# chao9527/Paddle_infer

Measured on AMD Instinct MI355X. Metric: tokens/sec (node) GPT-3 1.3B Fleet hybrid-parallel at 1/2/4/8 MI355X, higher is better.
Workload: dtype bf16; 1 GPU; model=GPT-3 1.3B, global_batch=96, seq_len=1024, parallelism=dp1, micro_batch_per_dp_rank=96, params=1313722368, optimizer=AdamW fp32 master, api=fleet.init/distributed_model/distributed_optimizer

## Files before the change

### paddle_infer_amd/csrc/kernels/layernorm.hip

```cpp
#include "common.h"

#include <cstdlib>
#include <type_traits>

namespace {

enum { DT_F32 = 0, DT_BF16 = 1, DT_F16 = 2 };

template <int DT>
struct IO16 {
  typedef unsigned short T;
  typedef u16x8 Raw;
  static __device__ __forceinline__ float cv(unsigned short v) {
    if (DT == DT_BF16) return bf2f(v);
    return (float)__builtin_bit_cast(_Float16, v);
  }
  static __device__ __forceinline__ unsigned short cvt(float f) {
    if (DT == DT_BF16) return f2bf(f);
    return __builtin_bit_cast(unsigned short, (_Float16)f);
  }
  static __device__ __forceinline__ Raw ldraw(const T* p) { return *reinterpret_cast<const Raw*>(p); }
  static __device__ __forceinline__ float el(const Raw& r, int j) { return cv(r[j]); }
  static __device__ __forceinline__ void load8(const T* p, float* v) {
    u16x8 r = *reinterpret_cast<const u16x8*>(p);
// ... 501 lines not shown
    __syncthreads();
    if (rp == 0) {
#pragma unroll
      for (int i = 0; i < NV; ++i) {
        const int vi = vcol(i);
        if (vi >= nvec) continue;
        f32x4 a, b;
#pragma unroll
        for (int j = 0; j < 4; ++j) {
          a[j] = (q == 0 ? dg[i][j] : (q == 1 ? db[i][j] : dbi[i][j])) + cmb[half][lane][i * 8 + j];
          b[j] = (q == 0 ? dg[i][4 + j] : (q == 1 ? db[i][4 + j] : dbi[i][4 + j])) + cmb[half][lane][i * 8 + 4 + j];
        }
        *reinterpret_cast<f32x4*>(outs[q] + srow + vi * 8) = a;
        *reinterpret_cast<f32x4*>(outs[q] + srow + vi * 8 + 4) = b;
      }
    }
    __syncthreads();
  }
}


#define LN_BWD_PAIR_PARAMS                                                                         \
  const typename IO<DT>::T *__restrict__ dy, const typename IO<DT>::T *__restrict__ h,             \
      const typename IO<DT>::T *__restrict__ gamma, const float *__restrict__ mean_in,             \
      const float *__restrict__ rstd_in, const typename IO<DT>::T *__restrict__ dres_in,           \
      typename IO<DT>::T *__restrict__ dres, typename IO<DT>::T *__restrict__ dx,                  \
      float *__restrict__ acc_dg, float *__restrict__ acc_db, float *__restrict__ acc_dbias, int rows, \
      int N, float p_drop, uint64_t seed, uint64_t offset, int rms
#define LN_BWD_PAIR_ARGS dy, h, gamma, mean_in, rstd_in, dres_in, dres, dx, acc_dg, acc_db, acc_dbias, \
                         rows, N, p_drop, seed, offset, rms
template <int DT>
__global__ __launch_bounds__(256) __attribute__((amdgpu_waves_per_eu(3, 3))) void ln_bwd_pair_kernel(
    LN_BWD_PAIR_PARAMS) {
  ln_bwd_pair_body<DT>(LN_BWD_PAIR_ARGS);
}
template <int DT>
__global__ __launch_bounds__(256) void ln_bwd_pair_kernel_f32(LN_BWD_PAIR_PARAMS) {
  ln_bwd_pair_body<DT>(LN_BWD_PAIR_ARGS);
}
#undef LN_BWD_PAIR_PARAMS
#undef LN_BWD_PAIR_ARGS
template <int NV, int DT>
__global__ __launch_bounds__(512) void ln_bwd_wide_kernel(
    const typename IO<DT>::T* __restrict__ dy, const typename IO<DT>::T* __restrict__ h,
    const typename IO<DT>::T* __restrict__ gamma, const float* __restrict__ mean_in,
    const float* __restrict__ rstd_in, const typename IO<DT>::T* __restrict__ dres_in,
    typename IO<DT>::T* __restrict__ dres, typename IO<DT>::T* __restrict__ dx,
    float* __restrict__ acc_dg, float* __restrict__ acc_db, float* __restrict__ acc_dbias,
    int rows, int N, float p_drop, uint64_t seed, uint64_t offset, int rms) {
  __shared__ float red[16];
  const int nvec = N >> 3;
  float dg[NV][8], db[NV][8], dbi[NV][8];
#pragma unroll
  for (int i = 0; i < NV; ++i)
#pragma unroll
    for (int j = 0; j < 8; ++j) { dg[i][j] = 0.f; db[i][j] = 0.f; dbi[i][j] = 0.f; }
  const float keep_scale = p_drop > 0.f ? 1.f / (1.f - p_drop) : 1.f;
  for (int row = blockIdx.x; row < rows; row += gridDim.x)
    ln_bwd_row<NV, DT, 512, 8>(dy, h, gamma, mean_in[row], rstd_in[row], dres_in, dres, dx,
                               (size_t)row * N, threadIdx.x, nvec, N, p_drop, keep_scale, seed,
                               offset, rms, dg, db, dbi, red);
  float* outs[3] = {acc_dg, acc_db, acc_dbias};
  const size_t srow = (size_t)blockIdx.x * N;
#pragma unroll
  for (int q = 0; q < 3; ++q) {
    if (!outs[q]) continue;
#pragma unroll
    for (int i = 0; i < NV; ++i) {
      const int vi = i * 512 + threadIdx.x;
      if (vi < nvec) {
        f32x4 a, b;
#pragma unroll
        for (int j = 0; j < 4; ++j) {
          a[j] = q == 0 ? dg[i][j] : (q == 1 ? db[i][j] : dbi[i][j]);
          b[j] = q == 0 ? dg[i][4 + j] : (q == 1 ? db[i][4 + j] : dbi[i][4 + j]);
        }
        *reinterpret_cast<f32x4*>(outs[q] + srow + vi * 8) = a;
        *reinterpret_cast<f32x4*>(outs[q] + srow + vi * 8 + 4) = b;
      }
    }
  }
}

__global__ __launch_bounds__(256) void slab_reduce_kernel(float* __restrict__ s0, float* __restrict__ s1,
                                                          float* __restrict__ s2, float* __restrict__ a0,
                                                          float* __restrict__ a1, float* __restrict__ a2,
                                                          int G, int N) {
  const int q = blockIdx.z;
  const float* slab = q == 0 ? s0 : (q == 1 ? s1 : s2);
  float* acc = q == 0 ? a0 : (q == 1 ? a1 : a2);
  if (!slab) return;
  const int c4 = blockIdx.x * 1024 + threadIdx.x * 4;
  if (c4 >= N) return;
  const int g0 = blockIdx.y * 16, g1 = min(g0 + 16, G);
  f32x4 s = {0.f, 0.f, 0.f, 0.f};
#pragma unroll 4
  for (int g = g0; g < g1; ++g) s += *reinterpret_cast<const f32x4*>(slab + (size_t)g * N + c4);
#pragma unroll
  for (int j = 0; j < 4; ++j) atomicAdd(acc + c4 + j, s[j]);
}

template <int DT>
__global__ __launch_bounds__(256) void col_sum_kernel(const float* __restrict__ part, int G, int N,
                                                     typename IO<DT>::T* __restrict__ out,
                                                     int accumulate) {
  const int cl = threadIdx.x & 63, rg = threadIdx.x >> 6;
  const int col = blockIdx.x * 64 + cl;
  float s = 0.f;
  if (col < N)
    for (int g = rg; g < G; g += 4) s += part[(size_t)g * N + col];
  __shared__ float red[4][64];
  red[rg][cl] = s;
  __syncthreads();
  if (rg == 0 && col < N) {
    float t = red[0][cl] + red[1][cl] + red[2][cl] + red[3][cl];
    if (accumulate) t += IO<DT>::load1(out + col);
    IO<DT>::store1(out + col, t);
  }
}

template <int DT>
int launch_fwd(const void* x, const void* bias, const void* residual, const void* gamma,
               const void* beta, void* y, void* residual_out, float* mean, float* rstd, int rows,
               int N, float eps, float p, uint64_t seed, uint64_t off, int rms, hipStream_t st) {
  typedef typename IO<DT>::T T;
#define ROW_ARGS (const T*)x, (const T*)bias, (const T*)residual, (const T*)gamma, (const T*)beta, \
                 (T*)y, (T*)residual_out, mean, rstd, N, eps, p, seed, off, rms
  if (N > 4096) {
    switch ((N / 8 + 511) / 512) {
      case 2: hipLaunchKernelGGL((ln_fwd_row_kernel<8, 2, DT>), dim3(rows), dim3(512), 0, st, ROW_ARGS); break;
      case 3: hipLaunchKernelGGL((ln_fwd_row_kernel<8, 3, DT>), dim3(rows), dim3(512), 0, st, ROW_ARGS); break;
      case 4: hipLaunchKernelGGL((ln_fwd_row_kernel<8, 4, DT>), dim3(rows), dim3(512), 0, st, ROW_ARGS); break;
      default: return (int)hipErrorInvalidValue;
    }
    return (int)hipGetLastError();
  }
  static const int row_max = [] {
    const char* e = getenv("PIAMD_LN_ROW_MAX");
    return e ? atoi(e) : 512;
  }();
  if (rows <= row_max) {
    switch ((N / 8 + 255) / 256) {
      case 1: hipLaunchKernelGGL((ln_fwd_row_kernel<4, 1, DT>), dim3(rows), dim3(256), 0, st, ROW_ARGS); break;
      case 2: hipLaunchKernelGGL((ln_fwd_row_kernel<4, 2, DT>), dim3(rows), dim3(256), 0, st, ROW_ARGS); break;
      default: return (int)hipErrorInvalidValue;
    }
    return (int)hipGetLastError();
  }
#undef ROW_ARGS
  const int nv = (N / 8 + 63) / 64;
  dim3 grid((rows + 3) / 4), block(256);
#define LNF(NVV)                                                                                  \
  hipLaunchKernelGGL((ln_fwd_kernel<NVV, DT>), grid, block, 0, st, (const T*)x, (const T*)bias, \
                     (const T*)residual, (const T*)gamma, (const T*)beta, (T*)y,               \
                     (T*)residual_out, mean, rstd, rows, N, eps, p, seed, off, rms);           \
  break;
  switch (nv) {
    case 1: LNF(1)
    case 2: LNF(2)
    case 3: LNF(3)
    case 4: LNF(4)
    case 5: case 6: LNF(6)
    case 7: case 8: LNF(8)
    default: return (int)hipErrorInvalidValue;
  }
#undef LNF
  return (int)hipGetLastError();
}

static inline bool bwd_pair(int N) {
  static const bool on = [] {
    const char* e = getenv("PIAMD_LN_BWD_PAIR");
    return !(e && e[0] == '0');
  }();
  return on && N > 1024 && N <= 2048;
}

static inline int bwd_grid(int rows, int N) {
  if (bwd_pair(N)) {
    const int g = (rows + 1) / 2;
    return g > 768 ? 768 : (g < 1 ? 1 : g);
  }
// ... 27 lines not shown
    else
      hipLaunchKernelGGL((ln_bwd_pair_kernel<DT>), grid, block, 0, st, BWD_ARGS);
    return (int)hipGetLastError();
  }
  switch ((N / 8 + 63) / 64) {
    case 1: hipLaunchKernelGGL((ln_bwd_kernel<1, DT>), grid, block, 0, st, BWD_ARGS); break;
    case 2: hipLaunchKernelGGL((ln_bwd_kernel<2, DT>), grid, block, 0, st, BWD_ARGS); break;
    case 3: hipLaunchKernelGGL((ln_bwd_kernel<3, DT>), grid, block, 0, st, BWD_ARGS); break;
    case 4: hipLaunchKernelGGL((ln_bwd_kernel<4, DT>), grid, block, 0, st, BWD_ARGS); break;
    default: return (int)hipErrorInvalidValue;
  }
#undef BWD_ARGS
  return (int)hipGetLastError();
}

template <int DT>
__global__ __launch_bounds__(256) void col_sum4_kernel(const float* __restrict__ part, int G, int N,
                                                      typename IO<DT>::T* __restrict__ out,
                                                      int accumulate) {
  const int q = threadIdx.x & 7, rg = threadIdx.x >> 3;
  const int col = blockIdx.x * 32 + 4 * q;
  f32x4 s = {0.f, 0.f, 0.f, 0.f};
  if (col < N) {
#pragma unroll 4
    for (int g = rg; g < G; g += 32) s += *reinterpret_cast<const f32x4*>(part + (size_t)g * N + col);
  }
  __shared__ f32x4 red[32][9];
  red[rg][q] = s;
  __syncthreads();
  if (threadIdx.x < 32) {
    const int qq = threadIdx.x >> 2, j = threadIdx.x & 3, c = blockIdx.x * 32 + threadIdx.x;
    if (c < N) {
      float t = 0.f;
#pragma unroll 8
      for (int r = 0; r < 32; ++r) t += red[r][qq][j];
      if (accumulate) t += IO<DT>::load1(out + c);
      IO<DT>::store1(out + c, t);
    }
  }
}

template <int DT>
void launch_colsum_out(const float* part, int G, int N, void* out, int acc, hipStream_t st) {
  if (G >= 64 && N % 4 == 0 && ((uintptr_t)part & 15) == 0) {
    hipLaunchKernelGGL((col_sum4_kernel<DT>), dim3((N + 31) / 32), dim3(256), 0, st, part, G, N,
                       (typename IO<DT>::T*)out, acc);
    return;
  }
  hipLaunchKernelGGL((col_sum_kernel<DT>), dim3((N + 63) / 64), dim3(256), 0, st, part, G, N,
                     (typename IO<DT>::T*)out, acc);
}

}

PIAMD_EXPORT int piamd_layernorm_fwd(int dtype, const void* x, const void* bias,
                                     const void* residual, const void* gamma, const void* beta,
                                     void* y, void* residual_out, float* mean, float* rstd,
                                     int rows, int N, float eps, float p_drop, uint64_t seed,
                                     uint64_t offset, int flags, hipStream_t stream) {
  if (N % 8 != 0 || N > 16384 || dtype < 0 || dtype > 2) return (int)hipErrorInvalidValue;
  if (rows == 0) return 0;
  const int rms = flags & 1;
#define FWD(D) launch_fwd<D>(x, bias, residual, gamma, beta, y, residual_out, mean, rstd, rows, N, \
                             eps, p_drop, seed, offset, rms, stream)
  return dtype == DT_BF16 ? FWD(DT_BF16) : (dtype == DT_F16 ? FWD(DT_F16) : FWD(DT_F32));
#undef FWD
}

PIAMD_EXPORT long long piamd_layernorm_bwd_ws(int rows, int N) {
  return 3LL * ((long long)bwd_grid(rows, N) * N + N);
}

PIAMD_EXPORT int piamd_layernorm_bwd(int dtype, const void* dy, const void* h, const void* gamma,
                                     const float* mean, const float* rstd, const void* dres_in,
                                     void* dres, void* dx, void* dgamma, void* dbeta, void* dbias,
                                     float* ws, int rows, int N, float p_drop, uint64_t seed,
                                     uint64_t offset, int accum_mask, int flags,
                                     hipStream_t stream) {
  if (N % 8 != 0 || N > 16384 || dtype < 0 || dtype > 2) return (int)hipErrorInvalidValue;
  if (rows == 0) return 0;
  const int rms = flags & 1;
  const int G = bwd_grid(rows, N);
  void* outs[3] = {dgamma, dbeta, dbias};
  float *slab[3], *acc[3];
  for (int q = 0; q < 3; ++q) {
    slab[q] = outs[q] ? ws + (size_t)q * G * N : nullptr;
    acc[q] = outs[q] ? ws + (size_t)3 * G * N + (size_t)q * N : nullptr;
    if (outs[q]) (void)hipMemsetAsync(acc[q], 0, sizeof(float) * N, stream);
  }
#define BWD(D) launch_bwd<D>(dy, h, gamma, mean, rstd, dres_in, dres, dx, slab[0], slab[1], slab[2], \
                             rows, N, p_drop, seed, offset, rms, stream)
  int e = dtype == DT_BF16 ? BWD(DT_BF16) : (dtype == DT_F16 ? BWD(DT_F16) : BWD(DT_F32));
#undef BWD
  if (e) return e;
  if (dgamma || dbeta || dbias)
    hipLaunchKernelGGL(slab_reduce_kernel, dim3((N + 1023) / 1024, (G + 15) / 16, 3), dim3(256), 0,
                       stream, slab[0], slab[1], slab[2], acc[0], acc[1], acc[2], G, N);
  for (int q = 0; q < 3; ++q) {
    if (!outs[q]) continue;
    const int a = (accum_mask >> q) & 1;
    if (dtype == DT_BF16) launch_colsum_out<DT_BF16>(acc[q], 1, N, outs[q], a, stream);
    else if (dtype == DT_F16) launch_colsum_out<DT_F16>(acc[q], 1, N, outs[q], a, stream);
    else launch_colsum_out<DT_F32>(acc[q], 1, N, outs[q], a, stream);
  }
  return (int)hipGetLastError();
}

template <int DT>
__global__ __launch_bounds__(256) void rowsum_partial_kernel(const typename IO<DT>::T* __restrict__ x,
                                                            int rows, int N,
                                                            float* __restrict__ part) {
  const int col = blockIdx.y * 256 + threadIdx.x;
  if (col >= N) return;
  float s = 0.f;
  for (int r = blockIdx.x; r < rows; r += gridDim.x) {
    s += IO<DT>::load1(x + (size_t)r * N + col);
  }
  part[(size_t)blockIdx.x * N + col] = s;
}

__global__ __launch_bounds__(256) void rowsum_partial_bf16x8_kernel(const bf16_t* __restrict__ x,
                                                                    int rows, int N,
                                                                    float* __restrict__ part) {
  const int c8 = blockIdx.y * 256 + threadIdx.x;
  if (c8 * 8 >= N) return;
  float s[8] = {0, 0, 0, 0, 0, 0, 0, 0};
  constexpr int U = 4;
  for (int r0 = blockIdx.x; r0 < rows; r0 += U * gridDim.x) {
    u16x8 v[U];
#pragma unroll
    for (int u = 0; u < U; ++u) {
      const int r = min(r0 + u * (int)gridDim.x, rows - 1);
      v[u] = reinterpret_cast<const u16x8*>(x + (size_t)r * N)[c8];
    }
#pragma unroll
    for (int u = 0; u < U; ++u)
      if (r0 + u * (int)gridDim.x < rows)
#pragma unroll
        for (int j = 0; j < 8; ++j) s[j] += bf2f(v[u][j]);
  }
  float* p = part + (size_t)blockIdx.x * N + c8 * 8;
#pragma unroll
  for (int j = 0; j < 8; ++j) p[j] = s[j];
}

PIAMD_EXPORT int piamd_colsum(int dtype, const void* x, void* out, float* part, int G, int rows,
                              int N, int accumulate, hipStream_t stream) {
  if (rows == 0) return 0;
  if (dtype < 0 || dtype > 2) return (int)hipErrorInvalidValue;
  dim3 grid(G, (N + 255) / 256), block(256);
  if (dtype == DT_BF16 && N % 8 == 0)
    hipLaunchKernelGGL(rowsum_partial_bf16x8_kernel, dim3(G, (N / 8 + 255) / 256), block, 0, stream,
                       (const bf16_t*)x, rows, N, part);
  else if (dtype == DT_BF16)
    hipLaunchKernelGGL((rowsum_partial_kernel<DT_BF16>), grid, block, 0, stream, (const bf16_t*)x,
                       rows, N, part);
  else if (dtype == DT_F16)
    hipLaunchKernelGGL((rowsum_partial_kernel<DT_F16>), grid, block, 0, stream,
                       (const unsigned short*)x, rows, N, part);
  else
    hipLaunchKernelGGL((rowsum_partial_kernel<DT_F32>), grid, block, 0, stream, (const float*)x,
                       rows, N, part);
  if (dtype == DT_BF16) launch_colsum_out<DT_BF16>(part, G, N, out, accumulate, stream);
  else if (dtype == DT_F16) launch_colsum_out<DT_F16>(part, G, N, out, accumulate, stream);
  else launch_colsum_out<DT_F32>(part, G, N, out, accumulate, stream);
  return (int)hipGetLastError();
}

PIAMD_EXPORT int piamd_colsum_parts(int dtype, const float* part, int G, int N, void* out, int accumulate,
                                    hipStream_t stream) {
  if (G <= 0 || N <= 0) return 0;
  if (dtype == DT_BF16) launch_colsum_out<DT_BF16>(part, G, N, out, accumulate, stream);
  else if (dtype == DT_F16) launch_colsum_out<DT_F16>(part, G, N, out, accumulate, stream);
  else if (dtype == DT_F32) launch_colsum_out<DT_F32>(part, G, N, out, accumulate, stream);
  else return (int)hipErrorInvalidValue;
  return (int)hipGetLastError();
}
```

### paddle_infer_amd/csrc/kernels/xent.hip

```cpp
#include "common.h"

namespace {

__device__ __forceinline__ void online_update(float& m, float& s, float x) {
  if (x > m) { s = s * __expf(m - x) + 1.f; m = x; }
  else s += __expf(x - m);
}
__device__ __forceinline__ void online_merge(float& m, float& s, float m2, float s2) {
  float M = fmaxf(m, m2);
  if (M == -INFINITY) { m = M; s = 0.f; return; }
  s = s * __expf(m - M) + s2 * __expf(m2 - M);
  m = M;
}

template <int DT>
__global__ __launch_bounds__(256) void xent_stats_kernel(
    const void* __restrict__ logits, const long long* __restrict__ labels, int V,
    long long vocab_start, int ignore_index, float* __restrict__ out_max,
    float* __restrict__ out_sum, float* __restrict__ out_target) {
  constexpr bool BF16 = DT != 0, F16 = DT == 2;
  const int row = blockIdx.x;
  const size_t base = (size_t)row * V;
  float m = -INFINITY, s = 0.f;
  if (BF16 && (V % 8) == 0) {
    const u16x8* p = reinterpret_cast<const u16x8*>((const bf16_t*)logits + base);
    for (int i = threadIdx.x; i < V / 8; i += 256) {
      u16x8 r = p[i];
      float x[8], lm = -INFINITY;
#pragma unroll
      for (int j = 0; j < 8; ++j) { x[j] = h2f<F16>(r[j]); lm = fmaxf(lm, x[j]); }
      float ls = 0.f;
#pragma unroll
      for (int j = 0; j < 8; ++j) ls += __expf(x[j] - lm);
      online_merge(m, s, lm, ls);
    }
  } else {
    for (int i = threadIdx.x; i < V; i += 256) {
      float x = BF16 ? h2f<F16>(((const bf16_t*)logits)[base + i]) : ((const float*)logits)[base + i];
      online_update(m, s, x);
    }
  }
#pragma unroll
  for (int o = 32; o > 0; o >>= 1) {
    float m2 = __shfl_xor(m, o, 64), s2 = __shfl_xor(s, o, 64);
    online_merge(m, s, m2, s2);
  }
  __shared__ float sm[4], ss[4];
  const int lane = threadIdx.x & 63, w = threadIdx.x >> 6;
  if (lane == 0) { sm[w] = m; ss[w] = s; }
  __syncthreads();
  if (threadIdx.x == 0) {
    float M = sm[0], S = ss[0];
    for (int i = 1; i < 4; ++i) online_merge(M, S, sm[i], ss[i]);
    out_max[row] = M;
    out_sum[row] = S;
    const long long lab = labels[row];
    float t = 0.f;
    if (lab != ignore_index && lab >= vocab_start && lab < vocab_start + V) {
      const size_t k = base + (size_t)(lab - vocab_start);
      t = BF16 ? h2f<F16>(((const bf16_t*)logits)[k]) : ((const float*)logits)[k];
    }
    out_target[row] = t;
  }
}

template <int DT>
__global__ __launch_bounds__(256) void xent_bwd_kernel(
    const void* __restrict__ logits, const long long* __restrict__ labels,
    const float* __restrict__ lse, const float* __restrict__ dloss, float dloss_scalar, int V,
    long long vocab_start, int ignore_index, void* __restrict__ grad) {
  constexpr bool BF16 = DT != 0, F16 = DT == 2;
  const int row = blockIdx.x;
  const size_t base = (size_t)row * V;
  const long long lab = labels[row];
  const float L = lse[row];
  const float d = lab == ignore_index ? 0.f : (dloss ? dloss[row] : dloss_scalar);
  const long long tl = lab - vocab_start;
  if (BF16 && (V % 8) == 0) {
    const u16x8* p = reinterpret_cast<const u16x8*>((const bf16_t*)logits + base);
    u16x8* q = reinterpret_cast<u16x8*>((bf16_t*)grad + base);
    for (int i = threadIdx.x; i < V / 8; i += 256) {
      u16x8 r = p[i], o;
#pragma unroll
      for (int j = 0; j < 8; ++j) {
        float g = __expf(h2f<F16>(r[j]) - L);
        if ((long long)(i * 8 + j) == tl) g -= 1.f;
        o[j] = f2h<F16>(g * d);
      }
      q[i] = o;
    }
  } else {
    for (int i = threadIdx.x; i < V; i += 256) {
      float x = BF16 ? h2f<F16>(((const bf16_t*)logits)[base + i]) : ((const float*)logits)[base + i];
      float g = __expf(x - L);
      if ((long long)i == tl) g -= 1.f;
      g *= d;
      if (BF16) ((bf16_t*)grad)[base + i] = f2h<F16>(g);
      else ((float*)grad)[base + i] = g;
    }
  }
}

}

PIAMD_EXPORT int piamd_xent_stats(int dtype, const void* logits, const long long* labels, int rows,
                                  int V, long long vocab_start, int ignore_index, float* out_max,
                                  float* out_sum, float* out_target, hipStream_t stream) {
  if (rows == 0) return 0;
#define XS(D)                                                                                     \
  hipLaunchKernelGGL((xent_stats_kernel<D>), dim3(rows), dim3(256), 0, stream, logits, labels, V, \
                     vocab_start, ignore_index, out_max, out_sum, out_target)
  if (dtype == 1) XS(1); else if (dtype == 2) XS(2); else if (dtype == 0) XS(0);
  else return (int)hipErrorInvalidValue;
#undef XS
  return (int)hipGetLastError();
}

PIAMD_EXPORT int piamd_xent_bwd(int dtype, const void* logits, const long long* labels,
                                const float* lse, const float* dloss, float dloss_scalar, int rows,
                                int V, long long vocab_start, int ignore_index, void* grad,
                                hipStream_t stream) {
  if (rows == 0) return 0;
#define XB(D)                                                                                     \
  hipLaunchKernelGGL((xent_bwd_kernel<D>), dim3(rows), dim3(256), 0, stream, logits, labels, lse, \
                     dloss, dloss_scalar, V, vocab_start, ignore_index, grad)
  if (dtype == 1) XB(1); else if (dtype == 2) XB(2); else if (dtype == 0) XB(0);
  else return (int)hipErrorInvalidValue;
#undef XB
  return (int)hipGetLastError();
}
```

### paddle_infer_amd/models/gpt.py

```python
from __future__ import annotations

import math
from dataclasses import dataclass, field

import torch
import torch.nn.functional as F

from ..nn.layer.base import Layer, LayerList
from ..nn import initializer as I
from ..ops import fused_add_layer_norm, flash_attention_packed, bias_act, softmax_cross_entropy
from ..ops.linear import (_use_transposed, fused_mlp, fused_mlp_supported, mm_nt, transposed,
                          wgrad_into)
from ..ops.linear import linear as _linear
from ..ops.embedding import embedding as ops_embedding
from ..distributed.fleet.mp_layers import (ColumnParallelLinear, RowParallelLinear,
                                           VocabParallelEmbedding, c_identity)


@dataclass
class GPTConfig:
    vocab_size: int = 50304
    hidden_size: int = 2048
    num_layers: int = 24
    num_heads: int = 16
    num_kv_heads: int | None = None
    ffn_hidden_size: int | None = None
    max_position_embeddings: int = 1024
    hidden_dropout_prob: float = 0.1
    attention_probs_dropout_prob: float = 0.0
    layer_norm_eps: float = 1e-5
    initializer_range: float = 0.02
    activation: str = "gelu_tanh"
    tie_word_embeddings: bool = True
    dtype: str = "bfloat16"
    recompute: bool = False
    extra: dict = field(default_factory=dict)

    @property
    def head_dim(self):
        return self.hidden_size // self.num_heads

    @property
    def ffn(self):
        return self.ffn_hidden_size or 4 * self.hidden_size


PRESETS = {
    "gpt3-tiny": dict(vocab_size=1024, hidden_size=256, num_layers=2, num_heads=4,
                      max_position_embeddings=256),
    "gpt3-125m": dict(hidden_size=768, num_layers=12, num_heads=12),
    "gpt3-350m": dict(hidden_size=1024, num_layers=24, num_heads=16),
    "gpt3-760m": dict(hidden_size=1536, num_layers=24, num_heads=16),
    "gpt3-1.3b": dict(hidden_size=2048, num_layers=24, num_heads=16),
    "gpt3-2.7b": dict(hidden_size=2560, num_layers=32, num_heads=32),
    "gpt3-6.7b": dict(hidden_size=4096, num_layers=32, num_heads=32, max_position_embeddings=2048),
    "gpt3-13b": dict(hidden_size=5120, num_layers=40, num_heads=40, max_position_embeddings=2048),
}


def gpt_config(name: str, **over) -> GPTConfig:
    kw = dict(PRESETS[name])
    kw.update(over)
    return GPTConfig(**kw)


def _mp_size(group):
    import torch.distributed as dist
    return dist.get_world_size(group) if group is not None else 1


class GPTAttention(Layer):
    def __init__(self, cfg: GPTConfig, mp_group=None, layer_idx=0):
        super().__init__(dtype=cfg.dtype)
        t = _mp_size(mp_group)
        self.cfg = cfg
        self.heads = cfg.num_heads // t
        self.kv_heads = (cfg.num_kv_heads or cfg.num_heads) // t
        self.head_dim = cfg.head_dim
        qkv_out = (cfg.num_heads + 2 * (cfg.num_kv_heads or cfg.num_heads)) * cfg.head_dim
        std = cfg.initializer_range
        self.qkv_proj = ColumnParallelLinear(cfg.hidden_size, qkv_out, gather_output=False,
                                             mp_group=mp_group, dtype=cfg.dtype,
                                             weight_attr=I.Normal(0.0, std))
        self.out_proj = RowParallelLinear(cfg.hidden_size, cfg.hidden_size, input_is_parallel=True,
                                          mp_group=mp_group, dtype=cfg.dtype,
                                          weight_attr=I.Normal(0.0, std / math.sqrt(2 * cfg.num_layers)))
        self.mp_group = mp_group

    def forward(self, y):
        B, S, _ = y.shape
        x = c_identity(y, self.mp_group)
        qkv = _linear(x, self.qkv_proj.weight, self.qkv_proj.bias)
        qkv = qkv.view(B, S, self.heads + 2 * self.kv_heads, self.head_dim)
# ... 82 lines not shown
        return w + pe


class _LMHeadFn(torch.autograd.Function):

    @staticmethod
    def forward(ctx, y, w):
        shp = y.shape
        y2 = y.reshape(-1, shp[-1])
        ctx.save_for_backward(y2, w)
        ctx.shp = shp
        return mm_nt(y2.contiguous(), w).view(*shp[:-1], w.shape[0])

    @staticmethod
    def backward(ctx, dl):
        y2, w = ctx.saved_tensors
        dl2 = dl.reshape(-1, w.shape[0])
        dl2 = dl2.contiguous()
        if _use_transposed(dl2, w) or (dl2.is_cuda and dl2.dtype == w.dtype
                                       and dl2.dtype in (torch.bfloat16, torch.float16)):
            dy = mm_nt(dl2, transposed(w)).view(ctx.shp)
        else:
            dy = torch.mm(dl2, w).view(ctx.shp)
        mg = getattr(w, "main_grad", None)
        if mg is not None:
            wgrad_into(mg, dl2, y2)
            return dy, None
        return dy, wgrad_into(torch.zeros_like(w), dl2, y2)


class GPTModel(Layer):
    def __init__(self, cfg: GPTConfig, mp_group=None):
        super().__init__(dtype=cfg.dtype)
        self.cfg = cfg
        self.mp_group = mp_group
        self.embeddings = GPTEmbeddings(cfg, mp_group)
        self.layers = LayerList([GPTDecoderLayer(cfg, mp_group, i) for i in range(cfg.num_layers)])
        self.final_ln = _LNParams(cfg)

    def forward(self, input_ids, position_ids=None):
        emb = self.embeddings(input_ids, position_ids)
        p = self.cfg.hidden_dropout_prob if self.training else 0.0
        h = None
        out, bias = emb, None
        for layer in self.layers:
            if self.cfg.recompute and self.training:
                from ..distributed.fleet.recompute import recompute
                h, out = recompute(lambda hh, oo, bb, _l=layer: _l(hh, oo, bb)[:2], h, out, bias)
                bias = None if getattr(self, "_zero3", False) else layer.mlp.fc2.bias
            else:
                h, out, bias = layer(h, out, bias)
        y, _ = fused_add_layer_norm(out, h, self.final_ln.weight, self.final_ln.bias,
                                    self.cfg.layer_norm_eps, bias, p, self.training)
        return y


class GPTForPretraining(Layer):
    def __init__(self, cfg: GPTConfig, mp_group=None):
        super().__init__(dtype=cfg.dtype)
        self.cfg = cfg
        self.gpt = GPTModel(cfg, mp_group)
        self.mp_group = mp_group
        if not cfg.tie_word_embeddings:
            self.lm_head = self.create_parameter(
                [cfg.vocab_size // _mp_size(mp_group), cfg.hidden_size],
                default_initializer=I.Normal(0.0, cfg.initializer_range))

    @property
    def _stage3_persistent(self):
        return ["gpt.embeddings.word_embeddings"] if self.cfg.tie_word_embeddings else []

    def head_weight(self):
        if self.cfg.tie_word_embeddings:
            return self.gpt.embeddings.word_embeddings.weight
        return self.lm_head

    def forward(self, input_ids, labels=None, position_ids=None, loss_mask=None):
        y = self.gpt(input_ids, position_ids)
        y = c_identity(y, self.mp_group)
        logits = _LMHeadFn.apply(y, self.head_weight())
        if labels is None:
            return logits
        group = self.mp_group if _mp_size(self.mp_group) > 1 else None
        loss = softmax_cross_entropy(logits, labels, group=group, inplace_backward=True)
        if loss_mask is not None:
            lm = loss_mask.reshape(-1).float()
            return (loss.reshape(-1) * lm).sum() / lm.sum()
        return loss.float().mean()


class GPTPretrainingCriterion(Layer):

    def __init__(self, mp_group=None):
        super().__init__()
        self.mp_group = mp_group

    def forward(self, logits, labels, loss_mask=None):
        group = self.mp_group if _mp_size(self.mp_group) > 1 else None
        loss = softmax_cross_entropy(logits, labels, group=group)
        if loss_mask is None:
            return loss.float().mean()
        lm = loss_mask.reshape(-1).float()
        return (loss.reshape(-1).float() * lm).sum() / lm.sum()


def gpt_flops_per_token(cfg: GPTConfig, seq_len: int) -> float:
    h, L, V = cfg.hidden_size, cfg.num_layers, cfg.vocab_size
    per_layer = 2 * (3 * h * h + h * h + 2 * h * cfg.ffn) + 2 * 2 * seq_len * h / 2
    return 3 * (L * per_layer + 2 * h * V)


def _qkv_cols(cfg: GPTConfig):
    hk = cfg.num_kv_heads or cfg.num_heads
    D = cfg.head_dim
    return cfg.num_heads * D, hk * D


def shard_gpt_state_dict(full: dict, cfg: GPTConfig, rank: int, world: int) -> dict:
    out = {}
    qc, kc = _qkv_cols(cfg)
    for k, v in full.items():
        if k.endswith("qkv_proj.weight") or k.endswith("qkv_proj.bias"):
            q, kk, vv = v.split([qc, kc, kc], dim=-1)
            out[k] = torch.cat([t.chunk(world, dim=-1)[rank] for t in (q, kk, vv)], dim=-1).clone()
        elif k.endswith("fc1.weight") or k.endswith("fc1.bias"):
            out[k] = v.chunk(world, dim=-1)[rank].clone()
        elif k.endswith("out_proj.weight") or k.endswith("fc2.weight"):
            out[k] = v.chunk(world, dim=0)[rank].clone()
        elif k.endswith("word_embeddings.weight") or k == "lm_head":
            out[k] = v.chunk(world, dim=0)[rank].clone()
        else:
            out[k] = v.clone()
    return out


def merge_gpt_state_dicts(shards: list, cfg: GPTConfig) -> dict:
    world = len(shards)
    qc, kc = _qkv_cols(cfg)
    out = {}
    for k in shards[0]:
        vs = [s[k] for s in shards]
        if k.endswith("qkv_proj.weight") or k.endswith("qkv_proj.bias"):
            parts = [v.split([qc // world, kc // world, kc // world], dim=-1) for v in vs]
            out[k] = torch.cat([torch.cat([p[i] for p in parts], dim=-1) for i in range(3)], dim=-1)
        elif k.endswith("fc1.weight") or k.endswith("fc1.bias"):
            out[k] = torch.cat(vs, dim=-1)
        elif k.endswith("out_proj.weight") or k.endswith("fc2.weight") or \
                k.endswith("word_embeddings.weight") or k == "lm_head":
            out[k] = torch.cat(vs, dim=0)
        else:
            out[k] = vs[0]
    return out


class GPTEmbeddingPipe(GPTEmbeddings):

    @property
    def weight(self):
        return self.word_embeddings.weight

    def forward(self, input_ids, position_ids=None):
        return super().forward(input_ids, position_ids)


class GPTDecoderLayerPipe(GPTDecoderLayer):

# ... 89 lines not shown
```

### paddle_infer_amd/ops/__init__.py

```python
from .norm import layer_norm, fused_add_layer_norm, rms_norm, fused_add_rms_norm
from .attention import (flash_attention, flash_attention_packed, attention_reference,
                        flash_attention_varlen)
from .activation import bias_act, gelu, dropout, fused_softmax_mask
from .loss import softmax_cross_entropy
from .optim import adamw_flat, momentum_flat, sumsq
from . import _lib
from .inference import (qkv_prep, decode_attention, weight_quantize, weight_dequantize,
                        weight_only_linear, llm_int8_linear, int8_linear,
                        quantize_rows)


def _make_recordable():
    from ..static.framework import recordable
    g = globals()
    for name, ty in (("layer_norm", "layer_norm"), ("fused_add_layer_norm", "skip_layernorm"),
                     ("rms_norm", "rms_norm"), ("flash_attention", "flash_attn"),
                     ("flash_attention_packed", "flash_attn_packed"), ("bias_act", "fused_bias_act"),
                     ("gelu", "gelu"), ("dropout", "dropout"), ("fused_softmax_mask", "softmax_mask_fuse"),
                     ("softmax_cross_entropy", "softmax_with_cross_entropy"),
                     ("weight_only_linear", "weight_only_linear")):
        g[name] = recordable(ty)(g[name])


_make_recordable()
```

### paddle_infer_amd/ops/_lib.py

```python
from __future__ import annotations

import ctypes
import os
import threading

import torch

from .. import _build

_LIB = None
_LOCK = threading.Lock()

c_void_p, c_int, c_float, c_ll, c_u64 = (ctypes.c_void_p, ctypes.c_int, ctypes.c_float,
                                         ctypes.c_longlong, ctypes.c_uint64)

_SIGS = {
    "piamd_layernorm_fwd": [c_int, c_void_p, c_void_p, c_void_p, c_void_p, c_void_p, c_void_p,
                            c_void_p, c_void_p, c_void_p, c_int, c_int, c_float, c_float, c_u64,
                            c_u64, c_int, c_void_p],
    "piamd_layernorm_bwd": [c_int, c_void_p, c_void_p, c_void_p, c_void_p, c_void_p, c_void_p,
                            c_void_p, c_void_p, c_void_p, c_void_p, c_void_p, c_void_p, c_int, c_int,
                            c_float, c_u64, c_u64, c_int, c_int, c_void_p],
    "piamd_colsum": [c_int, c_void_p, c_void_p, c_void_p, c_int, c_int, c_int, c_int, c_void_p],
    "piamd_adamw_flat": [c_void_p, c_void_p, c_void_p, c_void_p, c_int, c_void_p, c_ll, c_float,
                         c_void_p, c_float, c_float, c_float, c_float, c_float, c_float, c_void_p,
                         c_float, c_void_p],
    "piamd_momentum_flat": [c_void_p, c_void_p, c_void_p, c_int, c_void_p, c_ll, c_float,
                            c_void_p, c_float, c_float, c_int, c_void_p, c_void_p],
    "piamd_sumsq": [c_void_p, c_int, c_ll, c_void_p, c_void_p, c_int, c_void_p],
    "piamd_xent_stats": [c_int, c_void_p, c_void_p, c_int, c_int, c_ll, c_int, c_void_p, c_void_p,
                         c_void_p, c_void_p],
    "piamd_xent_bwd": [c_int, c_void_p, c_void_p, c_void_p, c_void_p, c_float, c_int, c_int, c_ll,
                       c_int, c_void_p, c_void_p],
    "piamd_bias_act_fwd": [c_int, c_int, c_void_p, c_void_p, c_void_p, c_void_p, c_ll, c_int, c_void_p],
    "piamd_bias_act_bwd_grid": [c_int],
    "piamd_bias_act_bwd": [c_int, c_int, c_void_p, c_void_p, c_void_p, c_void_p, c_void_p, c_void_p,
                           c_int, c_int, c_int, c_void_p],
    "piamd_softmax_fwd": [c_int, c_void_p, c_void_p, c_int, c_int, c_void_p, c_int, c_int, c_float,
                          c_void_p],
    "piamd_softmax_bwd": [c_int, c_void_p, c_void_p, c_void_p, c_int, c_int, c_float, c_void_p],
    "piamd_dropout": [c_int, c_void_p, c_void_p, c_ll, c_float, c_u64, c_u64, c_void_p],
    "piamd_qkv_prep": [c_void_p, c_ll, c_void_p, c_void_p, c_void_p, c_void_p, c_int, c_int,
                       c_int, c_int, c_int, c_int, c_int, c_int, c_float, c_void_p],
    "piamd_decode_attn": [c_void_p, c_ll, c_void_p, c_int, c_int, c_int, c_float, c_void_p,
                          c_void_p, c_void_p, c_int, c_int, c_int, c_int, c_int, c_int, c_int,
                          c_void_p, c_ll, c_float, c_void_p, c_void_p, c_void_p, c_ll, c_void_p],
    "piamd_wo_gemm": [c_int, c_void_p, c_ll, c_void_p, c_void_p, c_void_p, c_void_p, c_ll,
                      c_void_p, c_void_p, c_int, c_int, c_int, c_int, c_int, c_void_p],
    "piamd_conv_wprep": [c_int, c_int, c_void_p, c_void_p, c_void_p, c_int, c_int, c_int, c_int, c_int,
                         c_int, c_int, c_void_p],
    "piamd_wo_gemm_ex": [c_int, c_void_p, c_ll, c_void_p, c_void_p, c_void_p, c_void_p, c_ll,
                         c_void_p, c_void_p, c_int, c_int, c_int, c_int, c_int, c_void_p,
                         c_void_p, c_float, c_void_p, c_ll, c_void_p],
    "piamd_wo_dequant": [c_int, c_void_p, c_void_p, c_void_p, c_int, c_int, c_void_p],
}


_RESTYPES = {"piamd_layernorm_bwd_ws": ctypes.c_longlong, "piamd_dconv2d_wgrad_parts": ctypes.c_longlong,
             "piamd_group_norm_ws": ctypes.c_longlong}


class FaArgs(ctypes.Structure):
    _fields_ = ([(n, c_void_p) for n in ("q", "k", "v", "o", "lse", "dout", "delta", "dq", "dk", "dv",
                                        "mask", "cu_q", "cu_k")]
                + [(n, c_int) for n in ("B", "Sq", "Sk", "Hq", "Hk", "D", "ltot", "causal")]
                + [(n, c_ll) for n in ("sqb", "sqs", "sqh", "skb", "sks", "skh", "svb", "svs", "svh",
                                       "sob", "sos", "soh", "smb", "smh", "smq")]
                + [("scale", ctypes.c_float), ("p_drop", ctypes.c_float), ("seed", c_u64),
                   ("offset", c_u64), ("map", c_int), ("ds", c_void_p)])


class MegaArgs(ctypes.Structure):
    _fields_ = ([("layers", c_void_p)] + [(n, c_int) for n in ("nl", "maxS", "nsplit", "act")]
                + [("eps", ctypes.c_float), ("scale_log2", ctypes.c_float)]
                + [(n, c_void_p) for n in ("resid", "rbuf", "qn", "kvn", "part", "h", "bar", "err",
                                        "pos", "trace")] + [("late_dma", c_int), ("loader", c_int)]
                + [("rot", c_int), ("neox", c_int), ("log2_base", ctypes.c_float), ("w8", c_int),
                   ("nb", c_int), ("mm", c_int)])


_SIGS["piamd_decode_mega"] = [ctypes.POINTER(MegaArgs), c_int, c_int, c_int, c_int, c_int, c_void_p]
_SIGS["piamd_decode_mega_shape_supported"] = [c_int] * 7
_SIGS["piamd_decode_mega_batch_supported"] = [c_int] * 8
_SIGS["piamd_decode_mega_variant_supported"] = [c_int] * 9


class HeadArgs(ctypes.Structure):
    _fields_ = ([(n, c_void_p) for n in ("y", "g", "b")] + [("eps", ctypes.c_float), ("V", c_int)]
                + [(n, c_void_p) for n in ("w", "best", "cnt", "out", "done")]
                + [("eos", ctypes.c_longlong), ("pad", ctypes.c_longlong)]
                + [(n, c_void_p) for n in ("pos", "tok", "wemb", "pemb")]
                + [("P", c_int), ("resid", c_void_p)])


_SIGS["piamd_decode_head_greedy"] = [ctypes.POINTER(HeadArgs), c_int, c_void_p]
_SIGS["piamd_decode_mega_supported"] = []
_SIGS["piamd_fa_fwd"] = [ctypes.POINTER(FaArgs), c_int, c_void_p]
_SIGS["piamd_fa_bwd"] = [ctypes.POINTER(FaArgs), c_int, c_void_p]
_SIGS["piamd_layernorm_bwd_ws"] = [c_int, c_int]


def lib_path() -> str:
    return os.environ.get("PIAMD_KERNEL_LIB") or _build.KERNEL_LIB


def _load():
    global _LIB
    with _LOCK:
        if _LIB is not None:
            return _LIB
        path = lib_path()
        if not os.path.exists(path):
            raise RuntimeError(
                f"paddle_infer_amd HIP kernel library not built ({path}); run "
                "`python -m paddle_infer_amd._build` (or __graft_entry__.build()).")
        lib = ctypes.CDLL(path, mode=ctypes.RTLD_GLOBAL)
# ... 168 lines not shown
```

### paddle_infer_amd/ops/loss.py

```python
from __future__ import annotations

import torch
import torch.distributed as dist
import torch.nn.functional as F

from . import _lib


def _stats(logits2, labels, vocab_start, ignore_index):
    rows, V = logits2.shape
    m = torch.empty(rows, device=logits2.device, dtype=torch.float32)
    s = torch.empty_like(m)
    t = torch.empty_like(m)
    _lib.call("piamd_xent_stats", _lib.dtype_code(logits2, fp16=True), logits2.data_ptr(), labels.data_ptr(),
              rows, V, int(vocab_start), int(ignore_index), m.data_ptr(), s.data_ptr(), t.data_ptr(),
              _lib.stream())
    return m, s, t


class _XentFn(torch.autograd.Function):
    @staticmethod
    def forward(ctx, logits, labels, ignore_index, group, inplace_backward):
        V = logits.shape[-1]
        lg = logits.contiguous().view(-1, V)
        lab = labels.contiguous().view(-1).to(torch.int64)
        vocab_start = 0
        if group is not None:
            vocab_start = dist.get_rank(group) * V
        m, s, t = _stats(lg, lab, vocab_start, ignore_index)
        if group is not None:
            M = m.clone()
            dist.all_reduce(M, op=dist.ReduceOp.MAX, group=group)
            s = s * torch.exp(m - M)
            dist.all_reduce(s, group=group)
            dist.all_reduce(t, group=group)
            m = M
        lse = torch.log(s) + m
        valid = lab != ignore_index
        loss = torch.where(valid, lse - t, torch.zeros_like(lse))
        ctx.save_for_backward(lg, lab, lse)
        ctx.meta = (ignore_index, vocab_start, inplace_backward, logits.shape)
        return loss.view(labels.shape)

    @staticmethod
    def backward(ctx, dloss):
        lg, lab, lse = ctx.saved_tensors
        ignore_index, vocab_start, inplace, shp = ctx.meta
        rows, V = lg.shape
        d = dloss.contiguous().view(-1).float()
        grad = lg if inplace else torch.empty_like(lg)
        _lib.call("piamd_xent_bwd", _lib.dtype_code(lg, fp16=True), lg.data_ptr(), lab.data_ptr(), lse.data_ptr(),
                  d.data_ptr(), 0.0, rows, V, int(vocab_start), int(ignore_index), grad.data_ptr(),
                  _lib.stream())
        return grad.view(shp), None, None, None, None


def _reference(logits, labels, ignore_index):
    V = logits.shape[-1]
    x = logits.float() if logits.element_size() < 4 else logits
    return F.cross_entropy(x.reshape(-1, V), labels.reshape(-1).long(),
                           ignore_index=ignore_index, reduction="none").view(labels.shape)


def softmax_cross_entropy(logits, labels, ignore_index: int = -100, group=None,
                          inplace_backward: bool = False):
    if logits.is_cuda and logits.dtype in (torch.bfloat16, torch.float16, torch.float32):
        return _XentFn.apply(logits, labels, ignore_index, group, inplace_backward)
    if group is not None and dist.get_world_size(group) > 1:
        return _parallel_reference(logits, labels, ignore_index, group)
    return _reference(logits, labels, ignore_index)


def vocab_parallel_softmax_xent(logits, labels, ignore_index=-100, group=None, rank=None):
    V = logits.shape[-1]
    lg = logits.reshape(-1, V)
    lab = labels.reshape(-1).to(torch.int64)
    if rank is None:
        rank = dist.get_rank(group) if group is not None else 0
    start = int(rank) * V
    if lg.is_cuda and lg.dtype in (torch.bfloat16, torch.float16, torch.float32):
        lgc = lg.contiguous()
        m, s, t = _stats(lgc, lab, start, ignore_index)
    else:
        x = lg.float()
        m = x.max(dim=-1).values
        s = torch.exp(x - m[:, None]).sum(-1)
        inr = (lab >= start) & (lab < start + V)
        idx = torch.where(inr, lab - start, torch.zeros_like(lab))
        t = torch.gather(x, -1, idx[:, None]).squeeze(-1) * inr
    if group is not None and dist.get_world_size(group) > 1:
        M = m.clone()
        dist.all_reduce(M, op=dist.ReduceOp.MAX, group=group)
        s = s * torch.exp(m - M)
        dist.all_reduce(s, group=group)
        dist.all_reduce(t, group=group)
        m = M
    lse = torch.log(s) + m
    loss = torch.where(lab != ignore_index, lse - t, torch.zeros_like(lse))
    softmax = torch.exp(lg.float() - lse[:, None]).to(logits.dtype)
    return softmax.reshape(logits.shape), loss.reshape(labels.shape)


def _parallel_reference(logits, labels, ignore_index, group):
    V = logits.shape[-1]
    rank = dist.get_rank(group)
    start = rank * V
    x = logits.float()
    m = x.max(dim=-1).values.detach()
    M = _AllReduceMax.apply(m, group)
    e = torch.exp(x - M.unsqueeze(-1))
    s = _AllReduceSum.apply(e.sum(-1), group)
    lab = labels.long()
    inr = (lab >= start) & (lab < start + V)
    idx = torch.where(inr, lab - start, torch.zeros_like(lab))
    t = torch.gather(x, -1, idx.unsqueeze(-1)).squeeze(-1) * inr
    t = _AllReduceSum.apply(t, group)
    loss = torch.log(s) + M - t
    return torch.where(lab != ignore_index, loss, torch.zeros_like(loss))


class _AllReduceSum(torch.autograd.Function):
    @staticmethod
    def forward(ctx, x, group):
        y = x.clone()
        dist.all_reduce(y, group=group)
        return y

    @staticmethod
    def backward(ctx, g):
        return g, None


class _AllReduceMax(torch.autograd.Function):
    @staticmethod
    def forward(ctx, x, group):
        y = x.clone()
        dist.all_reduce(y, op=dist.ReduceOp.MAX, group=group)
        return y

    @staticmethod
    def backward(ctx, g):
        return torch.zeros_like(g), None
```

Baseline: 143,200 tokens/s.

## Fuse cross-entropy forward with in-place gradient and single-pass layernorm bwd finalize

Adds a fused cross-entropy kernel that computes the row softmax statistics and writes the gradient in place into the logits during the forward pass, holding each row in registers. Backward then only rescales the gradient by the upstream value, and skips even that when the upstream value is 1. This removes the separate stats pass and the re-read of the large vocabulary logits in backward. Separately, the layernorm backward parameter-gradient reduction (memset, atomic slab reduce, per-output colsum) is replaced by one finalize kernel per output that reduces the partial slabs in shared memory. The risk is that the logits are destroyed in forward, so anything else that reads them afterwards would see gradients, and the register-resident path adds register pressure.

```diff
diff --git a/paddle_infer_amd/csrc/kernels/layernorm.hip b/paddle_infer_amd/csrc/kernels/layernorm.hip
--- a/paddle_infer_amd/csrc/kernels/layernorm.hip
+++ b/paddle_infer_amd/csrc/kernels/layernorm.hip
@@ -607,22 +607,35 @@
   }
 }
 
-__global__ __launch_bounds__(256) void slab_reduce_kernel(float* __restrict__ s0, float* __restrict__ s1,
-                                                          float* __restrict__ s2, float* __restrict__ a0,
-                                                          float* __restrict__ a1, float* __restrict__ a2,
-                                                          int G, int N) {
-  const int q = blockIdx.z;
-  const float* slab = q == 0 ? s0 : (q == 1 ? s1 : s2);
-  float* acc = q == 0 ? a0 : (q == 1 ? a1 : a2);
-  if (!slab) return;
-  const int c4 = blockIdx.x * 1024 + threadIdx.x * 4;
-  if (c4 >= N) return;
-  const int g0 = blockIdx.y * 16, g1 = min(g0 + 16, G);
+template <int DT>
+__global__ __launch_bounds__(256) void ln_bwd_finalize_kernel(
+    const float* __restrict__ s0, const float* __restrict__ s1, const float* __restrict__ s2,
+    typename IO<DT>::T* __restrict__ o0, typename IO<DT>::T* __restrict__ o1,
+    typename IO<DT>::T* __restrict__ o2, int G, int N, int accum_mask) {
+  const int oq = blockIdx.y;
+  const float* part = oq == 0 ? s0 : (oq == 1 ? s1 : s2);
+  typename IO<DT>::T* out = oq == 0 ? o0 : (oq == 1 ? o1 : o2);
+  if (!out) return;
+  const int q = threadIdx.x & 7, rg = threadIdx.x >> 3;
+  const int col = blockIdx.x * 32 + 4 * q;
   f32x4 s = {0.f, 0.f, 0.f, 0.f};
-#pragma unroll 4
-  for (int g = g0; g < g1; ++g) s += *reinterpret_cast<const f32x4*>(slab + (size_t)g * N + c4);
-#pragma unroll
-  for (int j = 0; j < 4; ++j) atomicAdd(acc + c4 + j, s[j]);
+  if (col < N) {
+#pragma unroll 8
+    for (int g = rg; g < G; g += 32) s += *reinterpret_cast<const f32x4*>(part + (size_t)g * N + col);
+  }
+  __shared__ f32x4 red[32][9];
+  red[rg][q] = s;
+  __syncthreads();
+  if (threadIdx.x < 32) {
+    const int qq = threadIdx.x >> 2, j = threadIdx.x & 3, c = blockIdx.x * 32 + threadIdx.x;
+    if (c < N) {
+      float t = 0.f;
+#pragma unroll 8
+      for (int r = 0; r < 32; ++r) t += red[r][qq][j];
+      if ((accum_mask >> oq) & 1) t += IO<DT>::load1(out + c);
+      IO<DT>::store1(out + c, t);
+    }
+  }
 }
 
 template <int DT>
@@ -816,27 +829,20 @@
   const int rms = flags & 1;
   const int G = bwd_grid(rows, N);
   void* outs[3] = {dgamma, dbeta, dbias};
-  float *slab[3], *acc[3];
-  for (int q = 0; q < 3; ++q) {
-    slab[q] = outs[q] ? ws + (size_t)q * G * N : nullptr;
-    acc[q] = outs[q] ? ws + (size_t)3 * G * N + (size_t)q * N : nullptr;
-    if (outs[q]) (void)hipMemsetAsync(acc[q], 0, sizeof(float) * N, stream);
-  }
+  float* slab[3];
+  for (int q = 0; q < 3; ++q) slab[q] = outs[q] ? ws + (size_t)q * G * N : nullptr;
 #define BWD(D) launch_bwd<D>(dy, h, gamma, mean, rstd, dres_in, dres, dx, slab[0], slab[1], slab[2], \
                              rows, N, p_drop, seed, offset, rms, stream)
   int e = dtype == DT_BF16 ? BWD(DT_BF16) : (dtype == DT_F16 ? BWD(DT_F16) : BWD(DT_F32));
 #undef BWD
   if (e) return e;
-  if (dgamma || dbeta || dbias)
-    hipLaunchKernelGGL(slab_reduce_kernel, dim3((N + 1023) / 1024, (G + 15) / 16, 3), dim3(256), 0,
-                       stream, slab[0], slab[1], slab[2], acc[0], acc[1], acc[2], G, N);
-  for (int q = 0; q < 3; ++q) {
-    if (!outs[q]) continue;
-    const int a = (accum_mask >> q) & 1;
-    if (dtype == DT_BF16) launch_colsum_out<DT_BF16>(acc[q], 1, N, outs[q], a, stream);
-    else if (dtype == DT_F16) launch_colsum_out<DT_F16>(acc[q], 1, N, outs[q], a, stream);
-    else launch_colsum_out<DT_F32>(acc[q], 1, N, outs[q], a, stream);
-  }
+  if (!(dgamma || dbeta || dbias)) return 0;
+#define FIN(D)                                                                                     \
+  hipLaunchKernelGGL((ln_bwd_finalize_kernel<D>), dim3((N + 31) / 32, 3), dim3(256), 0, stream,    \
+                     slab[0], slab[1], slab[2], (IO<D>::T*)dgamma, (IO<D>::T*)dbeta,               \
+                     (IO<D>::T*)dbias, G, N, accum_mask)
+  if (dtype == DT_BF16) FIN(DT_BF16); else if (dtype == DT_F16) FIN(DT_F16); else FIN(DT_F32);
+#undef FIN
   return (int)hipGetLastError();
 }
 
diff --git a/paddle_infer_amd/csrc/kernels/xent.hip b/paddle_infer_amd/csrc/kernels/xent.hip
--- a/paddle_infer_amd/csrc/kernels/xent.hip
+++ b/paddle_infer_amd/csrc/kernels/xent.hip
@@ -101,6 +101,145 @@
   }
 }
 
+constexpr int XENT_REG_VECS = 25;
+
+template <bool FMA>
+__device__ __forceinline__ void online_merge_pinned(float& m, float& s, float m2, float s2) {
+#pragma clang fp contract(off)
+  float M = fmaxf(m, m2);
+  if (M == -INFINITY) { m = M; s = 0.f; return; }
+  const float a = s * __expf(m - M), e2 = __expf(m2 - M);
+  s = FMA ? __builtin_fmaf(s2, e2, a) : a + s2 * e2;
+  m = M;
+}
+
+__device__ __forceinline__ float log_as_torch(float s) {
+  return (float)((double)__builtin_amdgcn_logf(s) * 0.6931471805599453);
+}
+
+template <int DT, bool REG>
+__global__ __launch_bounds__(256) void xent_fwd_grad_kernel(
+    void* logits, const long long* __restrict__ labels, int V, int ignore_index, float scale,
+    float* __restrict__ out_max, float* __restrict__ out_sum, float* __restrict__ out_target) {
+  constexpr bool BF16 = DT != 0, F16 = DT == 2;
+  static_assert(!REG || DT != 0, "the register-resident path holds 16-bit rows");
+  const int row = blockIdx.x;
+  const size_t base = (size_t)row * V;
+  const int nvec = V >> 3;
+  u16x8* p = reinterpret_cast<u16x8*>((bf16_t*)logits + base);
+  u16x8 r[REG ? XENT_REG_VECS : 1];
+  float m = -INFINITY, s = 0.f;
+  auto merge8 = [&](const u16x8& v) {
+    float x[8], lm = -INFINITY;
+#pragma unroll
+    for (int j = 0; j < 8; ++j) { x[j] = h2f<F16>(v[j]); lm = fmaxf(lm, x[j]); }
+    float ls = 0.f;
+#pragma unroll
+    for (int j = 0; j < 8; ++j) ls += __expf(x[j] - lm);
+    online_merge_pinned<false>(m, s, lm, ls);
+  };
+  if constexpr (REG) {
+#pragma unroll
+    for (int k = 0; k < XENT_REG_VECS; ++k) {
+      const int i = k * 256 + threadIdx.x;
+      if (i < nvec) r[k] = __builtin_nontemporal_load(p + i);
+    }
+#pragma unroll
+    for (int k = 0; k < XENT_REG_VECS; ++k)
+      if (k * 256 + (int)threadIdx.x < nvec) merge8(r[k]);
+  } else if (BF16 && (V % 8) == 0) {
+    for (int i = threadIdx.x; i < nvec; i += 256) merge8(p[i]);
+  } else {
+    for (int i = threadIdx.x; i < V; i += 256) {
+      float x = BF16 ? h2f<F16>(((const bf16_t*)logits)[base + i]) : ((const float*)logits)[base + i];
+      online_update(m, s, x);
+    }
+  }
+#pragma unroll
+  for (int o = 32; o > 0; o >>= 1) {
+    float m2 = __shfl_xor(m, o, 64), s2 = __shfl_xor(s, o, 64);
+    online_merge_pinned<true>(m, s, m2, s2);
+  }
+  __shared__ float sm[4], ss[4], slse;
+  const int lane = threadIdx.x & 63, w = threadIdx.x >> 6;
+  const long long lab = labels[row];
+  if (lane == 0) { sm[w] = m; ss[w] = s; }
+  __syncthreads();
+  if (threadIdx.x == 0) {
+    float M = sm[0], S = ss[0];
+    for (int i = 1; i < 4; ++i) online_merge_pinned<false>(M, S, sm[i], ss[i]);
+    float t = 0.f;
+    if (lab != ignore_index && lab >= 0 && lab < V) {
+      const size_t k = base + (size_t)lab;
+      t = BF16 ? h2f<F16>(((const bf16_t*)logits)[k]) : ((const float*)logits)[k];
+    }
+    out_max[row] = M;
+    out_sum[row] = S;
+    out_target[row] = t;
+    slse = log_as_torch(S) + M;
+  }
+  __syncthreads();
+  const float L = slse;
+  const float d = lab == ignore_index ? 0.f : scale;
+  if constexpr (REG) {
+#pragma unroll
+    for (int k = 0; k < XENT_REG_VECS; ++k) asm volatile("" : "+v"(r[k]));
+  }
+  auto grad8 = [&](const u16x8& v, int i) {
+    u16x8 o;
+#pragma unroll
+    for (int j = 0; j < 8; ++j) {
+      float g = __expf(h2f<F16>(v[j]) - L);
+      if ((long long)(i * 8 + j) == lab) g -= 1.f;
+      o[j] = f2h<F16>(g * d);
+    }
+    return o;
+  };
+  if constexpr (REG) {
+#pragma unroll
+    for (int k = 0; k < XENT_REG_VECS; ++k) {
+      const int i = k * 256 + threadIdx.x;
+      if (i < nvec) __builtin_nontemporal_store(grad8(r[k], i), p + i);
+    }
+  } else if (BF16 && (V % 8) == 0) {
+    for (int i = threadIdx.x; i < nvec; i += 256) p[i] = grad8(p[i], i);
+  } else {
+    for (int i = threadIdx.x; i < V; i += 256) {
+      float x = BF16 ? h2f<F16>(((const bf16_t*)logits)[base + i]) : ((const float*)logits)[base + i];
+      float g = __expf(x - L);
+      if ((long long)i == lab) g -= 1.f;
+      g *= d;
+      if (BF16) ((bf16_t*)logits)[base + i] = f2h<F16>(g);
+      else ((float*)logits)[base + i] = g;
+    }
+  }
+}
+
+template <int DT>
+__global__ __launch_bounds__(256) void xent_rescale_kernel(void* grad, const float* __restrict__ up,
+                                                          int rows, int V) {
+  constexpr bool BF16 = DT != 0, F16 = DT == 2;
+  const float u = *up;
+  if (u == 1.0f) return;
+  for (int row = blockIdx.x; row < rows; row += gridDim.x) {
+    const size_t base = (size_t)row * V;
+    if (BF16 && (V % 8) == 0) {
+      u16x8* p = reinterpret_cast<u16x8*>((bf16_t*)grad + base);
+      for (int i = threadIdx.x; i < V / 8; i += 256) {
+        u16x8 v = p[i];
+#pragma unroll
+        for (int j = 0; j < 8; ++j) v[j] = f2h<F16>(h2f<F16>(v[j]) * u);
+        p[i] = v;
+      }
+    } else {
+      for (int i = threadIdx.x; i < V; i += 256) {
+        if (BF16) ((bf16_t*)grad)[base + i] = f2h<F16>(h2f<F16>(((bf16_t*)grad)[base + i]) * u);
+        else ((float*)grad)[base + i] *= u;
+      }
+    }
+  }
+}
+
 }
 
 PIAMD_EXPORT int piamd_xent_stats(int dtype, const void* logits, const long long* labels, int rows,
@@ -129,3 +268,30 @@
 #undef XB
   return (int)hipGetLastError();
 }
+
+PIAMD_EXPORT int piamd_xent_fwd_grad(int dtype, void* logits, const long long* labels, int rows,
+                                     int V, int ignore_index, float scale, float* out_max,
+                                     float* out_sum, float* out_target, hipStream_t stream) {
+  if (rows == 0) return 0;
+  if (dtype < 0 || dtype > 2 || V <= 0) return (int)hipErrorInvalidValue;
+  const bool reg = dtype != 0 && V % 8 == 0 && V / 8 <= XENT_REG_VECS * 256;
+#define XF(D, R)                                                                                 \
+  hipLaunchKernelGGL((xent_fwd_grad_kernel<D, R>), dim3(rows), dim3(256), 0, stream, logits,     \
+                     labels, V, ignore_index, scale, out_max, out_sum, out_target)
+  if (dtype == 1) { if (reg) XF(1, true); else XF(1, false); }
+  else if (dtype == 2) { if (reg) XF(2, true); else XF(2, false); }
+  else XF(0, false);
+#undef XF
+  return (int)hipGetLastError();
+}
+
+PIAMD_EXPORT int piamd_xent_rescale(int dtype, void* grad, const float* upstream, int rows, int V,
+                                    hipStream_t stream) {
+  if (rows == 0) return 0;
+  if (dtype < 0 || dtype > 2 || V <= 0) return (int)hipErrorInvalidValue;
+  const dim3 grid(rows < 4096 ? rows : 4096), block(256);
+#define XR(D) hipLaunchKernelGGL((xent_rescale_kernel<D>), grid, block, 0, stream, grad, upstream, rows, V)
+  if (dtype == 1) XR(1); else if (dtype == 2) XR(2); else XR(0);
+#undef XR
+  return (int)hipGetLastError();
+}
diff --git a/paddle_infer_amd/models/gpt.py b/paddle_infer_amd/models/gpt.py
--- a/paddle_infer_amd/models/gpt.py
+++ b/paddle_infer_amd/models/gpt.py
@@ -8,7 +8,8 @@
 
 from ..nn.layer.base import Layer, LayerList
 from ..nn import initializer as I
-from ..ops import fused_add_layer_norm, flash_attention_packed, bias_act, softmax_cross_entropy
+from ..ops import (fused_add_layer_norm, flash_attention_packed, bias_act, softmax_cross_entropy,
+                   softmax_cross_entropy_mean)
 from ..ops.linear import (_use_transposed, fused_mlp, fused_mlp_supported, mm_nt, transposed,
                           wgrad_into)
 from ..ops.linear import linear as _linear
@@ -257,6 +258,8 @@
         if labels is None:
             return logits
         group = self.mp_group if _mp_size(self.mp_group) > 1 else None
+        if loss_mask is None and group is None:
+            return softmax_cross_entropy_mean(logits, labels)
         loss = softmax_cross_entropy(logits, labels, group=group, inplace_backward=True)
         if loss_mask is not None:
             lm = loss_mask.reshape(-1).float()
diff --git a/paddle_infer_amd/ops/__init__.py b/paddle_infer_amd/ops/__init__.py
--- a/paddle_infer_amd/ops/__init__.py
+++ b/paddle_infer_amd/ops/__init__.py
@@ -2,7 +2,7 @@
 from .attention import (flash_attention, flash_attention_packed, attention_reference,
                         flash_attention_varlen)
 from .activation import bias_act, gelu, dropout, fused_softmax_mask
-from .loss import softmax_cross_entropy
+from .loss import softmax_cross_entropy, softmax_cross_entropy_mean
 from .optim import adamw_flat, momentum_flat, sumsq
 from . import _lib
 from .inference import (qkv_prep, decode_attention, weight_quantize, weight_dequantize,
diff --git a/paddle_infer_amd/ops/_lib.py b/paddle_infer_amd/ops/_lib.py
--- a/paddle_infer_amd/ops/_lib.py
+++ b/paddle_infer_amd/ops/_lib.py
@@ -32,6 +32,9 @@
                          c_void_p, c_void_p],
     "piamd_xent_bwd": [c_int, c_void_p, c_void_p, c_void_p, c_void_p, c_float, c_int, c_int, c_ll,
                        c_int, c_void_p, c_void_p],
+    "piamd_xent_fwd_grad": [c_int, c_void_p, c_void_p, c_int, c_int, c_int, c_float, c_void_p,
+                            c_void_p, c_void_p, c_void_p],
+    "piamd_xent_rescale": [c_int, c_void_p, c_void_p, c_int, c_int, c_void_p],
     "piamd_bias_act_fwd": [c_int, c_int, c_void_p, c_void_p, c_void_p, c_void_p, c_ll, c_int, c_void_p],
     "piamd_bias_act_bwd_grid": [c_int],
     "piamd_bias_act_bwd": [c_int, c_int, c_void_p, c_void_p, c_void_p, c_void_p, c_void_p, c_void_p,
diff --git a/paddle_infer_amd/ops/loss.py b/paddle_infer_amd/ops/loss.py
--- a/paddle_infer_amd/ops/loss.py
+++ b/paddle_infer_amd/ops/loss.py
@@ -71,6 +71,46 @@
     return _reference(logits, labels, ignore_index)
 
 
+class _XentMeanFn(torch.autograd.Function):
+
+    @staticmethod
+    def forward(ctx, logits, labels, ignore_index):
+        V = logits.shape[-1]
+        lg = logits.view(-1, V)
+        lab = labels.contiguous().view(-1).to(torch.int64)
+        rows = lg.shape[0]
+        m = torch.empty(rows, device=lg.device, dtype=torch.float32)
+        s = torch.empty_like(m)
+        t = torch.empty_like(m)
+        scale = (torch.ones((), dtype=torch.float32) / rows).item() if rows else 0.0
+        _lib.call("piamd_xent_fwd_grad", _lib.dtype_code(lg, fp16=True), lg.data_ptr(), lab.data_ptr(),
+                  rows, V, int(ignore_index), scale, m.data_ptr(), s.data_ptr(), t.data_ptr(),
+                  _lib.stream())
+        lse = torch.log(s) + m
+        valid = lab != ignore_index
+        loss = torch.where(valid, lse - t, torch.zeros_like(lse))
+        ctx.save_for_backward(lg)
+        ctx.shp = logits.shape
+        return loss.view(labels.shape).float().mean()
+
+    @staticmethod
+    def backward(ctx, dloss):
+        lg, = ctx.saved_tensors
+        rows, V = lg.shape
+        d = dloss.contiguous().float()
+        _lib.call("piamd_xent_rescale", _lib.dtype_code(lg, fp16=True), lg.data_ptr(), d.data_ptr(),
+                  rows, V, _lib.stream())
+        return lg.view(ctx.shp), None, None
+
+
+def softmax_cross_entropy_mean(logits, labels, ignore_index: int = -100, group=None):
+    if (group is None and logits.is_cuda and logits.is_contiguous()
+            and logits.dtype in (torch.bfloat16, torch.float16, torch.float32)
+            and torch.is_grad_enabled() and logits.requires_grad):
+        return _XentMeanFn.apply(logits, labels, ignore_index)
+    return softmax_cross_entropy(logits, labels, ignore_index, group).float().mean()
+
+
 def vocab_parallel_softmax_xent(logits, labels, ignore_index=-100, group=None, rank=None):
     V = logits.shape[-1]
     lg = logits.reshape(-1, V)
```

Result: no change. 143,700 tokens/s (median of 6 runs) (+0.4%).
